# heli-sudoo/HKD-MPC

Hardware: NVIDIA B200
Metric: batched HS-DDP solves/sec (higher is better)
Workload: dtype f64

## Files before the change

### hkd-mpc_b200/__init__.py

```python
import ctypes as C
import os
import subprocess
import numpy as np

_HERE = os.path.dirname(os.path.abspath(__file__))
LIB_PATH = os.environ.get("HSDDP_LIB") or os.path.join(_HERE, "libhsddp_b200.so")

MAX_PHASES = 16
MAX_STAGES = 128
TRACE_CAP = 64

STATUS_NAMES = {0: "converged", 1: "stalled", 2: "max_iter", 3: "reg_overflow"}

ARR = dict(Xbar=0, X=1, Defect=3, dX=4, G0=5, Ubar=10, U=11, dU=12, K=20, A=21, B=22, lxx=24, luu=25, H0=27,
           lx=30, lu=31, h=50, al=51, g=52, reb=53)


class HsddpError(RuntimeError):

    def __init__(self, msg, code=None):
        super().__init__(msg)
        self.code = code


# ... 97 lines not shown
        L.hsddp_batch_mpc_update.argtypes = [vp]
        L.hsddp_batch_last_update_ms.argtypes = [vp, C.POINTER(C.c_float)]
        L.hsddp_batch_restart_problems.argtypes = [vp, C.c_int, ip, ip, ip, dp, C.POINTER(Options)]
        L.hsddp_batch_get_schedule_ids.argtypes = [vp, ip]
        for f in ("hsddp_batch_solve", "hsddp_batch_solve_async", "hsddp_batch_compute_cost", "hsddp_batch_lq_approximation",
                  "hsddp_batch_prepare_merit", "hsddp_batch_update_al_params", "hsddp_batch_update_reb_params"):
            getattr(L, f).argtypes = [vp, C.POINTER(Options)]
        L.hsddp_batch_sync.argtypes = [vp]
        L.hsddp_batch_update_nominal.argtypes = [vp]
        L.hsddp_batch_last_solve_ms.argtypes = [vp, C.POINTER(C.c_float)]
        L.hsddp_batch_hybrid_rollout.argtypes = [vp, C.c_double, C.POINTER(Options), ip]
        L.hsddp_batch_backward_sweep.argtypes = [vp, C.c_double, ip]
        L.hsddp_batch_backward_sweep_regularized.argtypes = [vp, dp, C.POINTER(Options), ip]
        L.hsddp_batch_linear_rollout.argtypes = [vp, C.c_double, C.POINTER(Options)]
        L.hsddp_batch_forward_sweep.argtypes = [vp, C.POINTER(Options), ip, dp]
        L.hsddp_batch_dims.argtypes = [vp, ip, ip, ip]
        L.hsddp_batch_get_info.argtypes = [vp, vp]
        L.hsddp_batch_get_trace.argtypes = [vp, dp]
        L.hsddp_batch_get_scalars.argtypes = [vp, dp]
        L.hsddp_batch_get_array.argtypes = [vp, C.c_int, dp]
        L.hsddp_batch_set_array.argtypes = [vp, C.c_int, dp]
        L.hsddp_fp64_peak_tflops.argtypes = [C.c_int, C.c_int, dp]
        L.hsddp_batch_get_array_rows.argtypes = [vp, C.c_int, C.c_int, C.c_int, dp]
        L.hsddp_batch_get_gains_compact.argtypes = [vp, C.c_int, C.c_int, dp]
        L.hsddp_batch_get_mpc_command.argtypes = [vp, C.c_int, vp]
        L.hsddp_batch_set_problems_from_gaits.argtypes = [vp, C.c_int, ip, C.POINTER(C.c_float), dp, dp, dp, dp, ip, C.c_int, ip, ip, C.c_float, C.c_int, ip,
                                                          C.POINTER(ConstraintParams)]
        L.hsddp_batch_get_schedule.argtypes = [vp, C.c_int, ip, ip, ip, ip, dp, dp, dp, dp]
        L.hsddp_batch_set_solve_mode.argtypes = [vp, C.c_int]
        L.hsddp_batch_event_record.argtypes = [vp, C.c_int]
        L.hsddp_batch_event_elapsed_ms.argtypes = [vp, C.c_int, C.c_int, C.POINTER(C.c_float)]
        L.hsddp_batch_get_counters.argtypes = [vp, C.POINTER(C.c_ulonglong)]
        L.hsddp_batch_reset_counters.argtypes = [vp]
        L.hsddp_batch_get_profile.argtypes = [vp, C.POINTER(C.c_ulonglong)]
        L.hsddp_phase_batch_create.argtypes = [C.c_int] * 6 + [C.POINTER(vp)]
        L.hsddp_phase_batch_destroy.argtypes = [vp]
        L.hsddp_phase_batch_set.argtypes = [vp, C.c_int, dp]
        L.hsddp_phase_batch_backward_sweep.argtypes = [vp, C.c_double, dp, dp, ip]
        L.hsddp_phase_batch_linear_rollout.argtypes = [vp, C.c_double, dp]
        L.hsddp_phase_batch_set_gains.argtypes = [vp, dp, dp]
        L.hsddp_phase_batch_get.argtypes = [vp, C.c_int, dp]
        L.hsddp_phase_batch_last_ms.argtypes = [vp, C.POINTER(C.c_float)]
        _lib = L
    return _lib


def _dp(a):
    return a.ctypes.data_as(C.POINTER(C.c_double))


def _ip(a):
    return a.ctypes.data_as(C.POINTER(C.c_int32))


def _fp(a):
    return a.ctypes.data_as(C.POINTER(C.c_float))


def _check(rc, what):
    if rc != 0:
        raise HsddpError(f"{what} failed with code {rc}: {lib().hsddp_last_error().decode()}", rc)


def model_dynamics(x, u, dt, contact):
    x = np.ascontiguousarray(x, np.float64); u = np.ascontiguousarray(u, np.float64)
    c = np.ascontiguousarray(contact, np.int32); xn = np.zeros(24)
# ... 251 lines not shown

    def get_rows(self, name, row0, nrows, out=None):
        cols = {"K": 576, "g": 20, "h": 4, "al": 16, "reb": 40}.get(name, 24)
        if out is None:
            out = np.zeros((self.n, nrows, cols))
        _check(lib().hsddp_batch_get_array_rows(self.h, ARR[name], int(row0), int(nrows), _dp(out)), "get_array_rows")
        return out

    def get_gains_compact(self, row0, nrows, out=None):
        if out is None:
            out = np.zeros((self.n, nrows, 24, 12))
        _check(lib().hsddp_batch_get_gains_compact(self.h, int(row0), int(nrows), _dp(out)), "get_gains_compact")
        return out

    def mpc_command(self, n_steps=8, out=None):
        if out is None:
            out = np.zeros(self.n, dtype=CMD_DTYPE)
        _check(lib().hsddp_batch_get_mpc_command(self.h, int(n_steps), out.ctypes.data_as(C.c_void_p)), "get_mpc_command")
        return out

    def event_record(self, slot):
        _check(lib().hsddp_batch_event_record(self.h, int(slot)), "event_record")

    def event_elapsed_ms(self, slot0, slot1):
        ms = C.c_float()
        _check(lib().hsddp_batch_event_elapsed_ms(self.h, int(slot0), int(slot1), C.byref(ms)), "event_elapsed_ms")
        return ms.value

    def counters(self):
        out = (C.c_ulonglong * 4)()
        _check(lib().hsddp_batch_get_counters(self.h, out), "get_counters")
        return dict(sweep_stages=int(out[0]), solve_launches=int(out[1]), step_launches=int(out[2]))

    def profile(self):
        out = (C.c_ulonglong * 16)()
        _check(lib().hsddp_batch_get_profile(self.h, out), "get_profile")
        return [int(v) for v in out]

    def reset_counters(self):
        _check(lib().hsddp_batch_reset_counters(self.h), "reset_counters")

    def set(self, name, arr):
        arr = np.ascontiguousarray(arr, np.float64)
        if name == "K":
            arr = np.ascontiguousarray(np.swapaxes(arr, -1, -2))
        _check(lib().hsddp_batch_set_array(self.h, ARR[name], _dp(arr)), "set_array")



class SinglePhaseBatch:
    INPUTS = ["A", "B", "C", "D", "lx", "lu", "ly", "lxx", "luu", "lux", "lyy", "Phix", "Phixx", "Defect"]
    OUTPUTS = ["dU", "K", "G", "H", "dX", "dV"]
    _MATS = {"A", "B", "C", "D", "lxx", "luu", "lux", "lyy", "Phixx", "K", "H"}

    def __init__(self, xs, us, ys, horizon, n_problems, device=0):
        self.xs, self.us, self.ys, self.N, self.n = int(xs), int(us), int(ys), int(horizon), int(n_problems)
        self.h = C.c_void_p()
        _check(lib().hsddp_phase_batch_create(int(device), self.xs, self.us, self.ys, self.N, self.n, C.byref(self.h)), "hsddp_phase_batch_create")

    def __del__(self):
        try:
            if self.h:
                lib().hsddp_phase_batch_destroy(self.h)
        except Exception:
            pass

# ... 53 lines not shown
```

### hkd-mpc_b200/csrc/hsddp_device.cuh

```cuda
#pragma once
#include <cuda_runtime.h>
#include <stdint.h>
#include <cstddef>
#include "../../include/hsddp_b200.h"
#include "hkd_model.cuh"

#ifdef HSDDP_PROFILE
#define PROF_DECL long long prof_t0_ = clock64();
#define PROF_MARK(sm, slot)                                                         \
    do {                                                                            \
        if (threadIdx.x == 0) {                                                     \
            const long long t1_ = clock64();                                        \
            (sm).profacc[slot] += (unsigned long long)(t1_ - prof_t0_);             \
            prof_t0_ = t1_;                                                         \
        }                                                                           \
    } while (0)
#else
#define PROF_DECL
#define PROF_MARK(sm, slot) do { } while (0)
#endif

namespace hsddp {

constexpr int kThreads = 128;
// ... 21 lines not shown
constexpr int TQ_JC = 124;
constexpr int TQ_STRIDE = 200;

struct DevSchedule {
    int n_phases, n_stages, n_nodes, _pad;
    int horizon[MAXPH];
    int node_off[MAXPH];
    int stage_off[MAXPH];
    unsigned cmask[MAXPH];
    unsigned nmask[MAXPH];
    long long ref_off;
    double dt;
    unsigned char ph_of_stage[HSDDP_MAX_STAGES];
    unsigned char ph_of_node[HSDDP_MAX_STAGES + MAXPH];
    unsigned char ss_size[MAXPH];
    unsigned char tdmask[2][MAXPH];
};
static_assert(sizeof(DevSchedule) % 4 == 0, "bind_problem copies the schedule word by word");

struct SolverState {
    double actual_cost, merit, feas, dV_1, dV_2;
    double max_tconstr_prev, max_pconstr_prev, max_tconstr, max_pconstr, merit_rho;
    double reg;
    int rollout_ok, sweep_ok;
};

struct SolveCtl {
    int iter, iter_ou, iter_in, n_sweeps, n_trials, status;
    int active;
    int have_trial;
    int max_al, max_ddp;
    double cost0, feas0;
    double trial_cost, trial_feas;
};

struct BatchPtrs {
    int n_problems, max_stages, max_nodes, _pad;
    const DevSchedule* sched;
    const int* sched_id;
    const double *xr, *ur, *prel, *xinit;
    double* x0;
    double *Xbar, *X, *Xsim_t, *Defect, *dX;
    double *Ubar, *U, *U_t, *dU;
    double* KdX;
    double* K;
    double* lq;
    double* tq;
    double* gcon;
    double* reb;
    double* hcon;
    double* al;
    double* g0h0;
    SolverState* state;
    SolveCtl* ctl;
    const int* active;
    const int* n_active;
    int* next_active;
    int* next_count;
    int* zero_count;
    int sweep_w1_min;
    int lr_external;
    int _pad2;
    double *ls_X, *ls_Defect, *ls_Xsim, *ls_U, *ls_Ut, *ls_gcon, *ls_hcon, *ls_res;
    int* ls_mail;
    const int* order;
    const int* budget;
    hsddp_info* info;
    hsddp_iter_record* trace;
    unsigned long long* counters;
    int* work_counter;
    int* sm_slots;
    hsddp_constraint_params cp;
};

struct Smem;
struct __align__(16) Smem {
    double H[ro(24)], Y[ro(24)];
    double Z[zo(24)];
    double Qux[ro(16) + kQuuPad];
    double Quu[ro(12)];
    double rec[2][LQ_STRIDE];
    double dfc2[2][24];
    double G[24], Gn[24], Qx[24], Qu[24], wu[24], vtmp[24], vtmp2[24];
    double lxxd[24], lxxTd[24], lxxw[12], lxxTw[12];
    double swdt[4];
    double swc[16];
    double red[kThreads];
    DevSchedule sc;
    SolverState st;
    SolveCtl ctl;
    hsddp_constraint_params cp;
    hsddp_options opt;
    double *Xbar, *X, *Xsim_t, *Defect, *dX, *Ubar, *U, *U_t, *dU, *KdX, *K, *lqg, *tq, *gcon, *reb, *hcon, *al, *g0h0;
    const double *xr, *ur, *prel, *xinit, *x0;
    unsigned long long* prof;
    unsigned long long profacc[16];
    int pid;
    int rot;
    int flag;
    int ibuf[4];
    double dbuf[8];
};

static_assert(offsetof(Smem, dfc2) - offsetof(Smem, H) == sizeof(double) * kSweepDoubles, "kSweepDoubles must cover H..rec");
static_assert(32 * 113 <= kSweepDoubles, "LQ staging buffer does not fit");
// ... 682 lines not shown
```

### hkd-mpc_b200/csrc/hsddp_kernels.cu

```cuda
#include <cuda_runtime.h>
#include <cooperative_groups.h>
#include <cstdio>
#include <cstdlib>
#include <cstring>
#include <string>
#include <vector>
#include <map>
#include <algorithm>
#include "hsddp_device.cuh"
#include "hsddp_sweep.cuh"
#include "hsddp_sweep_w1.cuh"
#include "hsddp_lr_w1.cuh"

#ifndef HSDDP_MIN_BLOCKS
#define HSDDP_MIN_BLOCKS 6
#endif

namespace hsddp {

constexpr int hsddp_batch_max_groups = 16;

__device__ inline void prepare_merit_block(Smem& sm) {
    if (threadIdx.x == 0) {
        SolverState& st = sm.st;
// ... 191 lines not shown
    if (tid == 0) { sm.ctl.cost0 = sm.st.actual_cost; sm.ctl.feas0 = sm.st.feas; }
    __syncthreads();
    if (sm.ctl.max_al <= 0) {
        if (tid == 0) sm.ctl.active = 0;
        __syncthreads();
        return;
    }
    outer_start_block(sm);
    if (sm.ctl.max_ddp <= 0) outer_end_block(sm);
}

__device__ inline void iter_prep_block(Smem& sm, const BatchPtrs& bp) {
    if (sm.ctl.have_trial) {
        if (threadIdx.x == 0) { sm.st.actual_cost = sm.ctl.trial_cost; sm.st.feas = sm.ctl.trial_feas; }
        __syncthreads();
    } else {
        compute_cost_block(sm);
    }
    if (threadIdx.x == 0) {
        sm.ctl.iter_in++; sm.ctl.iter++;
        if (sm.ctl.iter <= HSDDP_TRACE_CAP) {
            hsddp_iter_record rec;
            rec.outer = sm.ctl.iter_ou; rec.inner = sm.ctl.iter_in; rec.cost_before = sm.st.actual_cost; rec.feas_before = sm.st.feas;
            rec.reg_after = rec.n_sweeps = 0;
            rec.dV_1 = rec.dV_2 = rec.merit_rho = rec.eps_accepted = rec.n_trials = 0; rec._pad = 0;
            rec.cost_after = rec.feas_after = rec.max_tconstr = rec.max_pconstr = 0;
            bp.trace[(size_t)sm.pid * HSDDP_TRACE_CAP + sm.ctl.iter - 1] = rec;
        }
    }
    __syncthreads();
    lq_approximation_block(sm);
}

__device__ inline void iter_sweep_block(Smem& sm, const BatchPtrs& bp) {
    int nsw = 0;
    const bool success = backward_sweep_regularized_block(sm, nsw);
    if (threadIdx.x == 0) {
        sm.ctl.n_sweeps += nsw;
        if (sm.ctl.iter <= HSDDP_TRACE_CAP) {
            hsddp_iter_record& rec = bp.trace[(size_t)sm.pid * HSDDP_TRACE_CAP + sm.ctl.iter - 1];
            rec.n_sweeps = nsw; rec.reg_after = sm.st.reg;
        }
        if (!success) { sm.ctl.status = HSDDP_STATUS_REG_OVERFLOW; sm.ctl.active = 0; }
    }
    __syncthreads();
}

template <bool CLUSTER_LS = false>
__device__ inline void iter_forward_block(Smem& sm, const BatchPtrs& bp) {
    const int tid = threadIdx.x;
    const hsddp_options& opt = sm.opt;
    hsddp_iter_record* rec = (sm.ctl.iter <= HSDDP_TRACE_CAP) ? bp.trace + (size_t)sm.pid * HSDDP_TRACE_CAP + sm.ctl.iter - 1 : nullptr;
    if (opt.MS && !bp.lr_external) linear_rollout_block(sm, 1.0);
    prepare_merit_block(sm);
    const double cost_prev = sm.st.actual_cost, merit_prev = sm.st.merit;
    const double dV_abs = fabs(sm.st.dV_1 + 0.5 * sm.st.dV_2);
    bool leave_inner = false;
    if (tid == 0 && rec) { rec->dV_1 = sm.st.dV_1; rec->dV_2 = sm.st.dV_2; rec->merit_rho = sm.st.merit_rho; }
    if ((dV_abs < opt.cost_thresh) && (sm.st.feas <= opt.dynamics_feas_thresh)) {
        if (tid == 0 && rec) {
            rec->eps_accepted = -1; rec->n_trials = 0;
            rec->cost_after = sm.st.actual_cost; rec->feas_after = sm.st.feas; rec->max_tconstr = sm.st.max_tconstr; rec->max_pconstr = sm.st.max_pconstr;
        }
        leave_inner = true;
    } else {
        double eps_acc = 0;
        int ntr = 0;
        if (CLUSTER_LS ? line_search_cluster(sm, bp, eps_acc, ntr) : line_search_block<true>(sm, eps_acc, ntr)) {
            update_nominal_block(sm);
        } else {
            __syncthreads();
            if (tid == 0) { sm.st.actual_cost = cost_prev; sm.st.merit = merit_prev; }
            __syncthreads();
        }
        if (tid == 0) {
            sm.ctl.n_trials += ntr;
            if (rec) {
                rec->eps_accepted = eps_acc; rec->n_trials = ntr;
// ... 105 lines not shown
                const int c = *rl.count[g];
                if (q < c) { pid = rl.list[g][q]; break; }
                q -= c;
            }
            sm.ibuf[3] = pid;
        }
        __syncthreads();
        const int pid = sm.ibuf[3];
        if (pid < 0) break;
        bind_problem(sm, bp, pid);
        if (threadIdx.x == 0) sm.opt = opt;
        __syncthreads();
        while (sm.ctl.active) {
            iter_prep_block(sm, bp);
            iter_sweep_block(sm, bp);
            if (!sm.ctl.active) break;
            iter_forward_block(sm, bp);
        }
        solve_finish_block(sm, bp);
        if (threadIdx.x == 0) { bp.state[pid] = sm.st; bp.ctl[pid] = sm.ctl; }
    }
}

enum SolvePhase { PH_BEGIN = 0, PH_PREP, PH_SWEEP, PH_FORWARD };
#ifndef HSDDP_MINB_SWEEP
#define HSDDP_MINB_SWEEP 5
#endif
#ifndef HSDDP_MINB_OTHER
#define HSDDP_MINB_OTHER 6
#endif
template <int PH>
__global__ void __launch_bounds__(kThreads, PH == 2 ? HSDDP_MINB_SWEEP : HSDDP_MINB_OTHER) k_phase(BatchPtrs bp, hsddp_options opt) {
    __shared__ Smem sm;
    if (PH == PH_PREP && bp.zero_count && blockIdx.x == 0 && threadIdx.x == 0) *bp.zero_count = 0;
    if (bp.n_active && (int)blockIdx.x >= *bp.n_active) return;
    if (PH == PH_SWEEP && bp.n_active && bp.sweep_w1_min > 0 && *bp.n_active >= bp.sweep_w1_min) return;
    const int pid = bp.active ? bp.active[blockIdx.x] : (int)blockIdx.x;
    if (threadIdx.x == 0) assign_rotation(bp.sm_slots, sm.rot);
    bind_problem(sm, bp, pid);
    if (threadIdx.x == 0) sm.opt = opt;
    __syncthreads();
#ifdef HSDDP_PROFILE
    if (threadIdx.x == 0) for (int i = 0; i < 16; ++i) sm.profacc[i] = 0;
    __syncthreads();
#endif
    if (PH == PH_BEGIN) solve_begin_block(sm, bp);
    if (PH == PH_PREP) iter_prep_block(sm, bp);
    if (PH == PH_SWEEP) iter_sweep_block(sm, bp);
    if (PH == PH_FORWARD) {
        if (sm.ctl.active) iter_forward_block(sm, bp);
    }
    __syncthreads();
    if (PH == PH_BEGIN || PH == PH_FORWARD) {
        if (sm.ctl.active) {
            if (threadIdx.x == 0) bp.next_active[atomicAdd(bp.next_count, 1)] = pid;
        } else {
            solve_finish_block(sm, bp);
        }
    }
    if (threadIdx.x == 0) { bp.state[pid] = sm.st; bp.ctl[pid] = sm.ctl; }
#ifdef HSDDP_PROFILE
    if (threadIdx.x == 0) for (int i = 0; i < 16; ++i) atomicAdd(&sm.prof[i], sm.profacc[i]);
#endif
}

enum StepOp { OP_RESET = 0, OP_ROLLOUT, OP_COST, OP_LQ, OP_SWEEP, OP_SWEEP_REG, OP_LINEAR, OP_MERIT, OP_FORWARD, OP_NOMINAL, OP_AL, OP_REB };

__global__ void __launch_bounds__(kThreads, HSDDP_MIN_BLOCKS) k_step(BatchPtrs bp, hsddp_options opt, int op, double arg, double* darg, int* ok) {
    __shared__ Smem sm;
    const int pid = blockIdx.x;
    if (threadIdx.x == 0) assign_rotation(bp.sm_slots, sm.rot);
    bind_problem(sm, bp, pid);
    if (threadIdx.x == 0) sm.opt = opt;
    __syncthreads();
    int okv = 1;
    switch (op) {
        case OP_RESET: cold_start_block(sm); break;
        case OP_ROLLOUT: okv = hybrid_rollout_block<false>(sm, arg) ? 1 : 0; break;
        case OP_COST: compute_cost_block(sm); break;
        case OP_LQ: lq_approximation_block(sm); break;
        case OP_SWEEP: okv = backward_sweep_block(sm, arg) ? 1 : 0; break;
        case OP_SWEEP_REG: {
            if (threadIdx.x == 0) sm.st.reg = darg[pid];
            __syncthreads();
            int nsw;
            okv = backward_sweep_regularized_block(sm, nsw) ? 1 : 0;
            if (threadIdx.x == 0) darg[pid] = sm.st.reg;
        } break;
        case OP_LINEAR: linear_rollout_block(sm, arg); break;
        case OP_MERIT: prepare_merit_block(sm); break;
        case OP_FORWARD: {
            const double cost_prev = sm.st.actual_cost, merit_prev = sm.st.merit;
            double eps_acc; int ntr;
// ... 440 lines not shown
namespace hsddp { void set_last_error(const std::string& s) { g_last_error = s; } }

#define CK(call)                                                                                   \
    do {                                                                                           \
        cudaError_t e_ = (call);                                                                   \
        if (e_ != cudaSuccess) {                                                                   \
            g_last_error = std::string(#call) + ": " + cudaGetErrorString(e_);                     \
            return HSDDP_ERR_CUDA;                                                                 \
        }                                                                                          \
    } while (0)

struct hsddp_batch {
    int device = 0;
    cudaStream_t stream = nullptr;
    cudaEvent_t ev0 = nullptr, ev1 = nullptr;
    cudaEvent_t slots[8] = {nullptr, nullptr, nullptr, nullptr, nullptr, nullptr, nullptr, nullptr};
    unsigned long long n_solve_launches = 0, n_step_launches = 0;
    int n_sm = 0, blocks_per_sm = 1;
    BatchPtrs bp{};
    std::vector<void*> allocs;
    std::vector<DevSchedule> h_sched;
    std::vector<int> h_sched_id;
    bool has_problems = false;
    bool cold = true;
    float last_ms = 0.f;
    int* d_ok = nullptr;
    double* d_darg = nullptr;
    int solve_mode = 0;
    int* d_active[2] = {nullptr, nullptr};
    int* d_count = nullptr;
    int last_rounds = 0;
    int sweep_kind = 2;
    int w1_min_blocks = 1036;
    bool lr_w1 = true;
    int* d_order = nullptr;
    bool have_order = false, use_order = true;
    bool cluster_ls = true;
    static constexpr int kClusterLsMax = 32;
    static constexpr int kMaxGroups = 16;
    int phased_min_group = 1024;
    int hybrid_rounds = 20, hybrid_groups = 4, hybrid_min_group = 256;
    int phased_groups = 4;
    cudaStream_t gstream[kMaxGroups] = {};
    cudaEvent_t gevent[kMaxGroups] = {};
    cudaEvent_t ev_fork = nullptr;
    hsddp_mpc_command* d_cmd = nullptr;
    bool mpc_ready = false;
    GaitLib lib{};
    int *d_sched_gait = nullptr, *d_sched_window = nullptr, *d_mpc_err = nullptr;
    MpcSched* d_mpc = nullptr;
    float plan = 0.f;
    int node_stride = 0, n_sched = 0;
    bool h_sched_stale = false;
    cudaEvent_t ev_u0 = nullptr, ev_u1 = nullptr;
    int n_gaits = 0;
    std::vector<int> slot_refs;
    std::vector<int> slot_free;
    int* d_restart = nullptr;
    double* d_restart_x0 = nullptr;
    size_t d_restart_cap = 0, d_restart_x0_cap = 0;
    int* d_budget = nullptr;
    long long budget_rounds = -1;
    bool slots_marked = false;
};

namespace {
// ... 108 lines not shown
        {(void**)&b->d_darg, 1, D, -1, 0},
    };
}

bool stored_array(hsddp_batch* b, int which, WsArray* out) {
    if (which < 0) return false;
    for (const WsArray& a : workspace_arrays(b))
        if (a.abi == which) { *out = a; return true; }
    return false;
}

struct SlotArray { void** field; size_t bytes; };

std::vector<SlotArray> slot_arrays(hsddp_batch* b) {
    BatchPtrs& bp = b->bp;
    const size_t rows = (size_t)b->node_stride, D = sizeof(double);
    return {
        {(void**)&bp.sched, sizeof(DevSchedule)}, {(void**)&b->d_mpc, sizeof(MpcSched)},
        {(void**)&b->d_sched_gait, sizeof(int)}, {(void**)&b->d_sched_window, sizeof(int)},
        {(void**)&bp.xr, 24 * rows * D}, {(void**)&bp.ur, 24 * rows * D}, {(void**)&bp.prel, 12 * rows * D}, {(void**)&bp.xinit, 24 * rows * D},
    };
}

void free_problem_allocs(hsddp_batch* b) {
    for (void* p : b->allocs) cudaFree(p);
    b->allocs.clear();
    b->d_cmd = nullptr;
    b->has_problems = false;
    b->mpc_ready = false;
    b->h_sched_stale = false;
    b->slot_refs.clear(); b->slot_free.clear();
    b->d_restart = nullptr; b->d_restart_x0 = nullptr; b->d_restart_cap = b->d_restart_x0_cap = 0;
    b->d_budget = nullptr; b->budget_rounds = -1;
    b->slots_marked = false;
}

hsddp_options default_options() {
    hsddp_options o;
    std::memset(&o, 0, sizeof o);
    o.alpha = 0.1; o.gamma = 0.01; o.update_penalty = 5; o.update_relax = 1; o.update_regularization = 2; o.update_ReB = 1;
    o.max_DDP_iter = 10; o.max_AL_iter = 5; o.cost_thresh = 1e-3; o.tconstr_thresh = 1e-3; o.pconstr_thresh = 1e-3;
    o.dynamics_feas_thresh = 1e-3; o.merit_scale = 0.2; o.merit_offset = 1e2; o.AL_active = 1; o.ReB_active = 1; o.MS = 1;
    return o;
}

const char* check_budget(int max_AL_iter, int max_DDP_iter) {
    if (max_DDP_iter < 0 || max_AL_iter < 0) return "max_DDP_iter / max_AL_iter must be >= 0";
    if ((long long)max_DDP_iter * (long long)max_AL_iter > 1000000LL) return "max_DDP_iter x max_AL_iter exceeds 1e6";
    return nullptr;
}

int check_opt(const hsddp_options* opt) {
    if (!opt) return HSDDP_OK;
    auto fin = [](double v) { return v == v && v - v == 0.0; };
    const char* bad = nullptr;
    if (!(opt->alpha > 0.0 && opt->alpha < 1.0)) bad = "alpha must be in (0, 1)";
    else if (!(opt->update_regularization > 1.0) || !fin(opt->update_regularization)) bad = "update_regularization must be finite and > 1";
    else if (!fin(opt->gamma) || !fin(opt->update_penalty) || !fin(opt->update_relax) || !fin(opt->update_ReB)) bad = "gamma / update_penalty / update_relax / update_ReB must be finite";
    else if (!fin(opt->cost_thresh) || !fin(opt->tconstr_thresh) || !fin(opt->pconstr_thresh) || !fin(opt->dynamics_feas_thresh)) bad = "thresholds must be finite";
    else if (!fin(opt->merit_scale) || opt->merit_scale == 1.0 || !fin(opt->merit_offset)) bad = "merit_scale must be finite and != 1, merit_offset finite";
    else bad = check_budget(opt->max_AL_iter, opt->max_DDP_iter);
    if (bad) { g_last_error = std::string("invalid hsddp_options: ") + bad; return HSDDP_ERR_ARG; }
    return HSDDP_OK;
}

int launch_step(hsddp_batch* b, const hsddp_options* opt, int op, double arg, double* darg_dev, int32_t* ok_host, bool sync = true) {
// ... 15 lines not shown

extern "C" {

static int batch_init(hsddp_batch* b, int device) {
    CK(cudaSetDevice(device));
    b->device = device;
    CK(cudaStreamCreateWithFlags(&b->stream, cudaStreamNonBlocking));
    CK(cudaEventCreate(&b->ev0));
    CK(cudaEventCreate(&b->ev1));
    CK(cudaEventCreate(&b->ev_u0));
    CK(cudaEventCreate(&b->ev_u1));
    for (int i = 0; i < 8; ++i) CK(cudaEventCreate(&b->slots[i]));
    cudaDeviceProp prop;
    CK(cudaGetDeviceProperties(&prop, device));
    b->n_sm = prop.multiProcessorCount;
    CK(cudaOccupancyMaxActiveBlocksPerMultiprocessor(&b->blocks_per_sm, k_solve, kThreads, 0));
    if (b->blocks_per_sm < 1) b->blocks_per_sm = 1;
    if (const char* e = getenv("HSDDP_BLOCKS_PER_SM")) {
        const int v = atoi(e);
        if (v >= 1 && v <= b->blocks_per_sm) b->blocks_per_sm = v;
    }
    CK(cudaEventCreateWithFlags(&b->ev_fork, cudaEventDisableTiming));
    if (const char* e = getenv("HSDDP_PHASED_GROUPS")) {
        const int v = atoi(e);
        if (v >= 1 && v <= hsddp_batch::kMaxGroups) b->phased_groups = v;
    }
    if (const char* e = getenv("HSDDP_PHASED_MIN_GROUP")) { const int v = atoi(e); if (v >= 1) b->phased_min_group = v; }
    if (const char* e = getenv("HSDDP_HYBRID_ROUNDS")) b->hybrid_rounds = atoi(e);
    if (const char* e = getenv("HSDDP_HYBRID_GROUPS")) { const int v = atoi(e); if (v >= 1 && v <= hsddp_batch::kMaxGroups) b->hybrid_groups = v; }
    if (const char* e = getenv("HSDDP_SWEEP_KIND")) b->sweep_kind = atoi(e);
    CK(cudaFuncSetAttribute(k_sweep_w1, cudaFuncAttributePreferredSharedMemoryCarveout, cudaSharedmemCarveoutMaxShared));
    CK(cudaFuncSetAttribute(k_lr_w1, cudaFuncAttributePreferredSharedMemoryCarveout, cudaSharedmemCarveoutMaxShared));
    if (const char* e = getenv("HSDDP_W1_MIN_BLOCKS")) b->w1_min_blocks = atoi(e);
    if (const char* e = getenv("HSDDP_LR_W1")) b->lr_w1 = atoi(e) != 0;
    if (const char* e = getenv("HSDDP_QUEUE_ORDER")) b->use_order = atoi(e) != 0;
    if (const char* e = getenv("HSDDP_CLUSTER_LS")) b->cluster_ls = atoi(e) != 0;
    if (const char* e = getenv("HSDDP_SOLVE_MODE")) {
        const int v = atoi(e);
        if (v >= 0 && v <= 3) b->solve_mode = v;
    }
    return HSDDP_OK;
}

int hsddp_batch_create(int device, hsddp_batch** out) {
    if (!out) return HSDDP_ERR_ARG;
    *out = nullptr;
    int n = 0;
    CK(cudaGetDeviceCount(&n));
    if (device < 0 || device >= n) { g_last_error = "no such CUDA device (this library has no CPU fallback)"; return HSDDP_ERR_CUDA; }
    return guarded([&]() -> int {
        hsddp_batch* b = new hsddp_batch();
        const int rc = batch_init(b, device);
        if (rc != HSDDP_OK) { hsddp_batch_destroy(b); return rc; }
        *out = b;
        return HSDDP_OK;
    });
}

int hsddp_batch_destroy(hsddp_batch* b) {
    if (!b) return HSDDP_OK;
    cudaSetDevice(b->device);
    free_problem_allocs(b);
    if (b->ev0) cudaEventDestroy(b->ev0);
    if (b->ev1) cudaEventDestroy(b->ev1);
    if (b->ev_u0) cudaEventDestroy(b->ev_u0);
    if (b->ev_u1) cudaEventDestroy(b->ev_u1);
// ... 398 lines not shown
    const int work = 33 * q.n_iter + 48 * q.n_sweeps + 12 * q.n_trials;
    return 255 - min(max(work >> 6, 0), 255);
}
__global__ void k_order_by_iterations(const hsddp_info* info, int n, int* order) {
    __shared__ int bins[256], start[256];
    for (int i = threadIdx.x; i < 256; i += blockDim.x) bins[i] = 0;
    __syncthreads();
    for (int i = threadIdx.x; i < n; i += blockDim.x) atomicAdd(&bins[order_bin(info[i])], 1);
    __syncthreads();
    if (threadIdx.x == 0) {
        int acc = 0;
        for (int i = 0; i < 256; ++i) { start[i] = acc; acc += bins[i]; }
    }
    __syncthreads();
    for (int bi = threadIdx.x; bi < 256; bi += blockDim.x) {
        if (!bins[bi]) continue;
        int pos = start[bi];
        for (int i = 0; i < n; ++i)
            if (order_bin(info[i]) == bi) order[pos++] = i;
    }
}

static int solve_phased(hsddp_batch* b, const hsddp_options& o, bool hybrid) {
    const int P = b->bp.n_problems;
    int G = hybrid ? b->hybrid_groups : b->phased_groups;
    G = std::min(G, std::max(1, P / (hybrid ? b->hybrid_min_group : b->phased_min_group)));
    G = std::max(1, std::min(G, hsddp_batch::kMaxGroups));
    for (int g = 0; g < G; ++g) {
        if (!b->gstream[g]) {
            CK(cudaStreamCreateWithFlags(&b->gstream[g], cudaStreamNonBlocking));
            CK(cudaEventCreateWithFlags(&b->gevent[g], cudaEventDisableTiming));
        }
    }
    CK(cudaEventRecord(b->ev0, b->stream));
    CK(cudaMemsetAsync(b->d_count, 0, 2 * hsddp_batch::kMaxGroups * sizeof(int), b->stream));
    k_iota<<<(P + 255) / 256, 256, 0, b->stream>>>(b->d_active[0], P);
    CK(cudaEventRecord(b->ev_fork, b->stream));
    const int all_rounds = (int)std::min<long long>(std::max((long long)std::max(0, o.max_AL_iter) * (long long)std::max(0, o.max_DDP_iter), b->budget_rounds), 1000000LL);
    const int rounds = hybrid ? std::min(all_rounds, std::max(0, b->hybrid_rounds)) : all_rounds;
    ResumeLists rl{};
    rl.n = 0;
    const bool use_block = b->sweep_kind != 1, use_w1 = b->sweep_kind != 0;
    int rc = HSDDP_OK;
    for (int g = 0; g < G && rc == HSDDP_OK; ++g) {
        const int lo = (int)((long long)P * g / G), n = (int)((long long)P * (g + 1) / G) - lo;
        if (n <= 0) continue;
        cudaStream_t st = b->gstream[g];
        int* cnt[2] = {b->d_count + 2 * g, b->d_count + 2 * g + 1};
        int* list[2] = {b->d_active[0] + lo, b->d_active[1] + lo};
        if (cudaStreamWaitEvent(st, b->ev_fork, 0) != cudaSuccess) { rc = HSDDP_ERR_CUDA; break; }
        BatchPtrs bp = b->bp;
        bp.sweep_w1_min = b->sweep_kind == 0 ? 0 : b->sweep_kind == 1 ? 1 : b->w1_min_blocks;
        bp.lr_external = (b->lr_w1 && o.MS) ? 1 : 0;
        bp.active = list[0]; bp.n_active = nullptr; bp.next_active = list[1]; bp.next_count = cnt[1]; bp.zero_count = nullptr;
        k_phase<PH_BEGIN><<<n, kThreads, 0, st>>>(bp, o);
        b->n_solve_launches++;
        for (int r = 1; r <= rounds; ++r) {
            const int cur = r & 1;
            bp.active = list[cur]; bp.n_active = cnt[cur]; bp.next_active = list[cur ^ 1]; bp.next_count = cnt[cur ^ 1]; bp.zero_count = cnt[cur ^ 1];
            k_phase<PH_PREP><<<n, kThreads, 0, st>>>(bp, o);
            if (use_block) k_phase<PH_SWEEP><<<n, kThreads, 0, st>>>(bp, o);
            if (use_w1) k_sweep_w1<<<n, 32, 0, st>>>(bp, o);
            if (bp.lr_external) k_lr_w1<<<n, 32, 0, st>>>(bp, o);
            k_phase<PH_FORWARD><<<n, kThreads, 0, st>>>(bp, o);
            b->n_solve_launches += 3 + (use_block && use_w1 ? 1 : 0) + (bp.lr_external ? 1 : 0);
        }
        if (cudaGetLastError() != cudaSuccess) { rc = HSDDP_ERR_CUDA; g_last_error = "kernel launch failed in the phased driver"; }
        const int nxt = (rounds + 1) & 1;
        rl.list[rl.n] = list[nxt]; rl.count[rl.n] = cnt[nxt]; rl.n++;
    }
    b->last_rounds = rounds;
    for (int g = 0; g < G; ++g) {
        if (!b->gstream[g]) continue;
        if (cudaEventRecord(b->gevent[g], b->gstream[g]) == cudaSuccess) cudaStreamWaitEvent(b->stream, b->gevent[g], 0);
    }
    if (hybrid && rounds < all_rounds && rc == HSDDP_OK) {
        CK(cudaMemsetAsync(b->bp.work_counter, 0, sizeof(int), b->stream));
        k_solve_resume<4><<<b->n_sm * 4, kThreads, 0, b->stream>>>(b->bp, o, rl);
        CK(cudaGetLastError());
        b->n_solve_launches++;
    }
    CK(cudaEventRecord(b->ev1, b->stream));
    return rc;
}

int hsddp_batch_set_solve_mode(hsddp_batch* b, int mode) {
    if (!b || mode < 0 || mode > 3) return HSDDP_ERR_ARG;
    b->solve_mode = mode;
    return HSDDP_OK;
}

static int consume_budget(hsddp_batch* b) {
    if (b->budget_rounds < 0) return HSDDP_OK;
    CK(cudaMemsetAsync(b->d_budget, 0xff, sizeof(int) * 2 * b->bp.n_problems, b->stream));
// ... 268 lines not shown
    }
    k_command<<<b->bp.n_problems, 128, 0, b->stream>>>(b->bp, n_steps, b->d_cmd);
    CK(cudaGetLastError());
    b->n_step_launches++;
    CK(cudaMemcpyAsync(out, b->d_cmd, bytes, cudaMemcpyDeviceToHost, b->stream));
    CK(cudaStreamSynchronize(b->stream));
    return HSDDP_OK;
}

int hsddp_batch_event_record(hsddp_batch* b, int slot) {
    if (!b || slot < 0 || slot >= 8) return HSDDP_ERR_ARG;
    CK(cudaSetDevice(b->device));
    CK(cudaEventRecord(b->slots[slot], b->stream));
    return HSDDP_OK;
}

int hsddp_batch_event_elapsed_ms(hsddp_batch* b, int slot0, int slot1, float* ms) {
    if (!b || !ms || slot0 < 0 || slot0 >= 8 || slot1 < 0 || slot1 >= 8) return HSDDP_ERR_ARG;
    CK(cudaSetDevice(b->device));
    CK(cudaEventSynchronize(b->slots[slot1]));
    CK(cudaEventElapsedTime(ms, b->slots[slot0], b->slots[slot1]));
    return HSDDP_OK;
}

int hsddp_batch_get_counters(hsddp_batch* b, unsigned long long out[4]) {
    if (!b || !b->has_problems || !out) return HSDDP_ERR_ARG;
    CK(cudaSetDevice(b->device));
    CK(cudaStreamSynchronize(b->stream));
    CK(cudaMemcpy(out, b->bp.counters, sizeof(unsigned long long), cudaMemcpyDeviceToHost));
    out[1] = b->n_solve_launches; out[2] = b->n_step_launches; out[3] = 0;
    return HSDDP_OK;
}

int hsddp_batch_get_profile(hsddp_batch* b, unsigned long long out[16]) {
    if (!b || !b->has_problems || !out) return HSDDP_ERR_ARG;
    CK(cudaSetDevice(b->device));
    CK(cudaStreamSynchronize(b->stream));
    CK(cudaMemcpy(out, b->bp.counters + 8, 16 * sizeof(unsigned long long), cudaMemcpyDeviceToHost));
    return HSDDP_OK;
}

int hsddp_batch_reset_counters(hsddp_batch* b) {
    if (!b || !b->has_problems) return HSDDP_ERR_ARG;
    CK(cudaSetDevice(b->device));
    CK(cudaMemsetAsync(b->bp.counters, 0, 32 * sizeof(unsigned long long), b->stream));
    b->n_solve_launches = 0; b->n_step_launches = 0;
    return HSDDP_OK;
}

int hsddp_fp64_peak_tflops(int device, int kind, double* tflops) {
    if (!tflops) return HSDDP_ERR_ARG;
    CK(cudaSetDevice(device));
    cudaDeviceProp prop;
    CK(cudaGetDeviceProperties(&prop, device));
    const int blocks = prop.multiProcessorCount * 8, threads = 256, iters = 20000;
    double* d = nullptr;
    CK(cudaMalloc(&d, sizeof(double) * blocks * threads));
    cudaEvent_t e0, e1;
    CK(cudaEventCreate(&e0));
    CK(cudaEventCreate(&e1));
    double best = 0;
    for (int rep = 0; rep < 4; ++rep) {
        CK(cudaEventRecord(e0));
        if (kind == 0) k_dfma_probe<<<blocks, threads>>>(d, iters);
        else k_dmma_probe<<<blocks, threads>>>(d, iters);
        CK(cudaEventRecord(e1));
// ... 16 lines not shown
```

### include/hsddp_b200.h

```cpp
#ifndef HSDDP_B200_H
#define HSDDP_B200_H

#include <stdint.h>

#ifdef __cplusplus
extern "C" {
#endif

#define HSDDP_NX 24
#define HSDDP_NU 24
#define HSDDP_MAX_PHASES 16
#define HSDDP_MAX_STAGES 128

#define HSDDP_OK 0
#define HSDDP_ERR_ARG (-1)
#define HSDDP_ERR_CUDA (-2)
#define HSDDP_ERR_UNSUPPORTED (-3)
#define HSDDP_ERR_STATE (-4)
#define HSDDP_ERR_IO (-5)

#define HSDDP_STATUS_CONVERGED 0
#define HSDDP_STATUS_STALLED 1
#define HSDDP_STATUS_MAX_ITER 2
#define HSDDP_STATUS_REG_OVERFLOW 3
// ... 119 lines not shown
#define HSDDP_ARR_LU 31
#define HSDDP_ARR_LUU 25
#define HSDDP_ARR_LXX 24
#define HSDDP_ARR_G0 5
#define HSDDP_ARR_H0 27
#define HSDDP_ARR_GCON 52
#define HSDDP_ARR_HCON 50
#define HSDDP_ARR_AL 51
#define HSDDP_ARR_REB 53
int hsddp_batch_get_array(hsddp_batch* b, int which, double* out);
int hsddp_batch_set_array(hsddp_batch* b, int which, const double* in);

int hsddp_batch_get_array_rows(hsddp_batch* b, int which, int row0, int nrows, double* out);

int hsddp_batch_get_gains_compact(hsddp_batch* b, int row0, int nrows, double* out);

#define HSDDP_CMD_MAX_STEPS 10
typedef struct hsddp_mpc_command {
    int32_t N_mpcsteps;
    int32_t foot_found[4];
    int32_t contacts[HSDDP_CMD_MAX_STEPS][4];
    float hkd_controls[HSDDP_CMD_MAX_STEPS][24];
    float des_body_state[HSDDP_CMD_MAX_STEPS][12];
    float feedback[HSDDP_CMD_MAX_STEPS][12][12];
    float foot_placement[12];
    int32_t _pad;
} hsddp_mpc_command;
int hsddp_batch_get_mpc_command(hsddp_batch* b, int n_steps, hsddp_mpc_command* out);

int hsddp_batch_event_record(hsddp_batch* b, int slot);
int hsddp_batch_event_elapsed_ms(hsddp_batch* b, int slot0, int slot1, float* ms);
int hsddp_batch_get_counters(hsddp_batch* b, unsigned long long out[4]);
int hsddp_batch_reset_counters(hsddp_batch* b);
int hsddp_batch_get_profile(hsddp_batch* b, unsigned long long out[16]);

typedef struct hsddp_phase_batch hsddp_phase_batch;
#define HSDDP_PH_A 0
#define HSDDP_PH_B 1
#define HSDDP_PH_C 2
#define HSDDP_PH_D 3
#define HSDDP_PH_LX 4
#define HSDDP_PH_LU 5
#define HSDDP_PH_LY 6
#define HSDDP_PH_LXX 7
#define HSDDP_PH_LUU 8
#define HSDDP_PH_LUX 9
#define HSDDP_PH_LYY 10
#define HSDDP_PH_PHIX 11
#define HSDDP_PH_PHIXX 12
#define HSDDP_PH_DEFECT 13
#define HSDDP_PH_N_INPUTS 14
#define HSDDP_PH_OUT_DU 0
#define HSDDP_PH_OUT_K 1
#define HSDDP_PH_OUT_G 2
#define HSDDP_PH_OUT_H 3
#define HSDDP_PH_OUT_DX 4
#define HSDDP_PH_OUT_DV 5
#define HSDDP_PH_N_OUTPUTS 6
int hsddp_phase_batch_create(int device, int xs, int us, int ys, int horizon, int n_problems, hsddp_phase_batch** out);
int hsddp_phase_batch_destroy(hsddp_phase_batch* b);
int hsddp_phase_batch_set(hsddp_phase_batch* b, int which, const double* host);
int hsddp_phase_batch_backward_sweep(hsddp_phase_batch* b, double regularization, const double* Gprime, const double* Hprime, int32_t* ok);
int hsddp_phase_batch_linear_rollout(hsddp_phase_batch* b, double eps, const double* dx_init);
int hsddp_phase_batch_set_gains(hsddp_phase_batch* b, const double* dU, const double* K);
int hsddp_phase_batch_get(hsddp_phase_batch* b, int which, double* host);
int hsddp_phase_batch_last_ms(hsddp_phase_batch* b, float* ms);
// ... 8 lines not shown
```

Measured before the change: 57150.

## Speculatively run regularization retries of backward sweep in parallel blocks

Problems likely to need regularization retries (nonzero reg or multiple sweeps last iteration) are flagged in the prep phase. The sweep kernel then launches extra blocks, each running the backward sweep at a higher candidate regularization level into scratch buffers. The last block to arrive picks the first successful candidate and copies its gains back. This turns serial retry sweeps into parallel ones, at the cost of extra blocks per round, scratch memory and atomics, and redundant work when the base sweep succeeds.

Measured after the change: 58950, median of 6. 1.03x the previous value.

```diff
diff --git a/hkd-mpc_b200/__init__.py b/hkd-mpc_b200/__init__.py
--- a/hkd-mpc_b200/__init__.py
+++ b/hkd-mpc_b200/__init__.py
@@ -153,6 +153,7 @@
         L.hsddp_batch_event_elapsed_ms.argtypes = [vp, C.c_int, C.c_int, C.POINTER(C.c_float)]
         L.hsddp_batch_get_counters.argtypes = [vp, C.POINTER(C.c_ulonglong)]
         L.hsddp_batch_reset_counters.argtypes = [vp]
+        L.hsddp_batch_get_speculation.argtypes = [vp, C.POINTER(C.c_ulonglong)]
         L.hsddp_batch_get_profile.argtypes = [vp, C.POINTER(C.c_ulonglong)]
         L.hsddp_phase_batch_create.argtypes = [C.c_int] * 6 + [C.POINTER(vp)]
         L.hsddp_phase_batch_destroy.argtypes = [vp]
@@ -470,6 +471,11 @@
         _check(lib().hsddp_batch_get_counters(self.h, out), "get_counters")
         return dict(sweep_stages=int(out[0]), solve_launches=int(out[1]), step_launches=int(out[2]))
 
+    def speculation(self):
+        out = (C.c_ulonglong * 3)()
+        _check(lib().hsddp_batch_get_speculation(self.h, out), "get_speculation")
+        return dict(rounds=int(out[0]), later=int(out[1]), exceeded=int(out[2]))
+
     def profile(self):
         out = (C.c_ulonglong * 16)()
         _check(lib().hsddp_batch_get_profile(self.h, out), "get_profile")
diff --git a/hkd-mpc_b200/csrc/hsddp_device.cuh b/hkd-mpc_b200/csrc/hsddp_device.cuh
--- a/hkd-mpc_b200/csrc/hsddp_device.cuh
+++ b/hkd-mpc_b200/csrc/hsddp_device.cuh
@@ -77,6 +77,11 @@
     int max_al, max_ddp;
     double cost0, feas0;
     double trial_cost, trial_feas;
+};
+
+struct SpecRec {
+    int ok, _pad;
+    double dV_1, dV_2;
 };
 
 struct BatchPtrs {
@@ -116,6 +121,14 @@
     int* work_counter;
     int* sm_slots;
     hsddp_constraint_params cp;
+    int* spec_list;
+    int* spec_count;
+    int* spec_zero;
+    int* spec_arrive;
+    int* spec_entry;
+    SpecRec* spec_rec;
+    double* spec_out;
+    int spec_S, spec_cap;
 };
 
 struct Smem;
diff --git a/hkd-mpc_b200/csrc/hsddp_kernels.cu b/hkd-mpc_b200/csrc/hsddp_kernels.cu
--- a/hkd-mpc_b200/csrc/hsddp_kernels.cu
+++ b/hkd-mpc_b200/csrc/hsddp_kernels.cu
@@ -247,9 +247,7 @@
     lq_approximation_block(sm);
 }
 
-__device__ inline void iter_sweep_block(Smem& sm, const BatchPtrs& bp) {
-    int nsw = 0;
-    const bool success = backward_sweep_regularized_block(sm, nsw);
+__device__ inline void finish_sweep_block(Smem& sm, const BatchPtrs& bp, bool success, int nsw) {
     if (threadIdx.x == 0) {
         sm.ctl.n_sweeps += nsw;
         if (sm.ctl.iter <= HSDDP_TRACE_CAP) {
@@ -259,6 +257,119 @@
         if (!success) { sm.ctl.status = HSDDP_STATUS_REG_OVERFLOW; sm.ctl.active = 0; }
     }
     __syncthreads();
+}
+
+__device__ inline void iter_sweep_block(Smem& sm, const BatchPtrs& bp) {
+    int nsw = 0;
+    const bool success = backward_sweep_regularized_block(sm, nsw);
+    finish_sweep_block(sm, bp, success, nsw);
+}
+
+__device__ __forceinline__ bool retry_reg(double& r, int j, double up) {
+    for (int i = 0; i < j; ++i) {
+        r = fmax(r * up, 1e-03);
+        if (r > 1e2) return false;
+    }
+    return true;
+}
+
+__device__ inline void spec_flag_block(Smem& sm, const BatchPtrs& bp) {
+    if (threadIdx.x == 0) {
+        const int row = sm.ctl.iter - 1;
+        bool flag = sm.st.reg > 0;
+        if (row >= 1 && row <= HSDDP_TRACE_CAP) flag = flag || bp.trace[(size_t)sm.pid * HSDDP_TRACE_CAP + row - 1].n_sweeps > 1;
+        int e = -1;
+        if (flag) {
+            e = atomicAdd(bp.spec_count, 1);
+            if (e < bp.spec_cap) bp.spec_list[e] = sm.pid;
+            else e = -1;
+        }
+        bp.spec_entry[sm.pid] = e;
+    }
+}
+
+constexpr unsigned long long kSpecUnwritten = 0x7ff0dead5eed0001ull;
+
+__device__ inline bool spec_commit_block(Smem& sm, const BatchPtrs& bp, int e, int j, bool ran, bool ok, double& reg, int& nsw, bool& success) {
+    const int tid = threadIdx.x, S = bp.spec_S, N = sm.sc.n_stages;
+    const size_t ms = (size_t)bp.max_stages, slice = ms * 312 + 600;
+    SpecRec* rec = bp.spec_rec + (size_t)e * S;
+    const double* out = bp.spec_out + (size_t)e * (S - 1) * slice;
+    if (tid == 0) rec[j] = SpecRec{ran ? (ok ? 1 : 0) : -1, 0, sm.st.dV_1, sm.st.dV_2};
+    __threadfence();
+    __syncthreads();
+    if (tid == 0) sm.ibuf[2] = atomicAdd(bp.spec_arrive + e, 1) == S - 1;
+    __syncthreads();
+    if (!sm.ibuf[2]) return false;
+    __threadfence();
+    if (tid == 0) {
+        bp.spec_arrive[e] = 0;
+        int w = -1, m = 0;
+        while (m < S) {
+            const int c = __ldcg(&rec[m].ok);
+            if (c < 0) break;
+            ++m;
+            if (c) { w = m - 1; break; }
+        }
+        const int c = w >= 0 ? w : m - 1;
+        sm.ibuf[2] = w; sm.ibuf[3] = m;
+        const size_t pid = (size_t)sm.pid;
+        sm.K = bp.K + pid * ms * 288; sm.dU = bp.dU + pid * ms * 24; sm.g0h0 = bp.g0h0 + pid * 600;
+        sm.st.dV_1 = __ldcg(&rec[c].dV_1); sm.st.dV_2 = __ldcg(&rec[c].dV_2); sm.st.sweep_ok = w >= 0 ? 1 : 0;
+        atomicAdd(bp.counters + 1, 1ull);
+        if (w != 0) atomicAdd(bp.counters + (w > 0 ? 2 : 3), 1ull);
+    }
+    __syncthreads();
+    const int w = sm.ibuf[2], m = sm.ibuf[3];
+    for (int c = (w >= 0 ? w : 1); c <= (w >= 0 ? w : m - 1); ++c) {
+        if (c == 0) continue;
+        const double* o = out + (c - 1) * slice;
+        const unsigned long long* mark = reinterpret_cast<const unsigned long long*>(o + ms * 288);
+        for (int x = tid; x < 288 * N; x += kThreads)
+            if (w >= 0 || __ldcg(mark + 24 * (x / 288)) != kSpecUnwritten) sm.K[x] = __ldcg(o + x);
+        for (int x = tid; x < 24 * N; x += kThreads)
+            if (w >= 0 || __ldcg(mark + 24 * (x / 24)) != kSpecUnwritten) sm.dU[x] = __ldcg(o + ms * 288 + x);
+        if (w >= 0)
+            for (int x = tid; x < 600; x += kThreads) sm.g0h0[x] = __ldcg(o + ms * 312 + x);
+        __syncthreads();
+    }
+    success = w >= 0;
+    nsw = success ? w + 1 : m;
+    reg = sm.st.reg;
+    retry_reg(reg, success ? w : m - 1, sm.opt.update_regularization);
+    return true;
+}
+
+__device__ inline bool sweep_round_block(Smem& sm, const BatchPtrs& bp, int e, int j) {
+    const int tid = threadIdx.x;
+    const double up = sm.opt.update_regularization;
+    double reg = sm.st.reg;
+    int nsw = 0;
+    bool success = false, run = e < 0 || retry_reg(reg, j, up);
+    if (e >= 0 && j > 0 && run) {
+        const size_t ms = (size_t)bp.max_stages;
+        double* o = bp.spec_out + ((size_t)e * (bp.spec_S - 1) + j - 1) * (ms * 312 + 600);
+        for (int s = tid; s < sm.sc.n_stages; s += kThreads) reinterpret_cast<unsigned long long*>(o + ms * 288)[24 * s] = kSpecUnwritten;
+        if (tid == 0) { sm.K = o; sm.dU = o + ms * 288; sm.g0h0 = o + ms * 312; }
+    }
+    __syncthreads();
+    for (;;) {
+        if (run) { ++nsw; success = backward_sweep_block(sm, reg); }
+        if (e >= 0) {
+            if (!spec_commit_block(sm, bp, e, j, run, success, reg, nsw, success)) return false;
+            e = -1;
+        }
+        if (success) break;
+        reg = fmax(reg * up, 1e-03);
+        if (reg > 1e2) break;
+        run = true;
+    }
+    reg = reg / 20;
+    if (reg < 1e-06) reg = 0;
+    if (tid == 0) sm.st.reg = reg;
+    __syncthreads();
+    finish_sweep_block(sm, bp, success, nsw);
+    return true;
 }
 
 template <bool CLUSTER_LS = false>
@@ -430,10 +541,20 @@
 template <int PH>
 __global__ void __launch_bounds__(kThreads, PH == 2 ? HSDDP_MINB_SWEEP : HSDDP_MINB_OTHER) k_phase(BatchPtrs bp, hsddp_options opt) {
     __shared__ Smem sm;
-    if (PH == PH_PREP && bp.zero_count && blockIdx.x == 0 && threadIdx.x == 0) *bp.zero_count = 0;
-    if (bp.n_active && (int)blockIdx.x >= *bp.n_active) return;
+    if (PH == PH_PREP && bp.zero_count && blockIdx.x == 0 && threadIdx.x == 0) {
+        *bp.zero_count = 0;
+        if (bp.spec_zero) *bp.spec_zero = 0;
+    }
+    int blk = (int)blockIdx.x, cand = 0, entry = -1;
+    if (PH == PH_SWEEP && bp.spec_list) {
+        const int ns = bp.spec_cap * (bp.spec_S - 1);
+        if (blk < ns) { entry = blk / (bp.spec_S - 1); cand = 1 + blk % (bp.spec_S - 1); }
+        blk -= ns;
+    }
+    if (bp.n_active && blk >= *bp.n_active) return;
     if (PH == PH_SWEEP && bp.n_active && bp.sweep_w1_min > 0 && *bp.n_active >= bp.sweep_w1_min) return;
-    const int pid = bp.active ? bp.active[blockIdx.x] : (int)blockIdx.x;
+    if (PH == PH_SWEEP && cand > 0 && entry >= min(*bp.spec_count, bp.spec_cap)) return;
+    const int pid = cand > 0 ? bp.spec_list[entry] : bp.active ? bp.active[blk] : blk;
     if (threadIdx.x == 0) assign_rotation(bp.sm_slots, sm.rot);
     bind_problem(sm, bp, pid);
     if (threadIdx.x == 0) sm.opt = opt;
@@ -442,9 +563,16 @@
     if (threadIdx.x == 0) for (int i = 0; i < 16; ++i) sm.profacc[i] = 0;
     __syncthreads();
 #endif
+    bool store = true;
     if (PH == PH_BEGIN) solve_begin_block(sm, bp);
-    if (PH == PH_PREP) iter_prep_block(sm, bp);
-    if (PH == PH_SWEEP) iter_sweep_block(sm, bp);
+    if (PH == PH_PREP) {
+        iter_prep_block(sm, bp);
+        if (bp.spec_list && (bp.sweep_w1_min == 0 || *bp.n_active < bp.sweep_w1_min)) spec_flag_block(sm, bp);
+    }
+    if (PH == PH_SWEEP) {
+        if (bp.spec_list && cand == 0) entry = bp.spec_entry[pid];
+        store = sweep_round_block(sm, bp, entry, cand);
+    }
     if (PH == PH_FORWARD) {
         if (sm.ctl.active) iter_forward_block(sm, bp);
     }
@@ -456,7 +584,7 @@
             solve_finish_block(sm, bp);
         }
     }
-    if (threadIdx.x == 0) { bp.state[pid] = sm.st; bp.ctl[pid] = sm.ctl; }
+    if (store && threadIdx.x == 0) { bp.state[pid] = sm.st; bp.ctl[pid] = sm.ctl; }
 #ifdef HSDDP_PROFILE
     if (threadIdx.x == 0) for (int i = 0; i < 16; ++i) atomicAdd(&sm.prof[i], sm.profacc[i]);
 #endif
@@ -963,6 +1091,12 @@
     int last_rounds = 0;
     int sweep_kind = 2;
     int w1_min_blocks = 1036;
+    int sweep_spec = 8;
+    static constexpr int kSpecCap = 128;
+    int* d_spec_int = nullptr;
+    SpecRec* d_spec_rec = nullptr;
+    double* d_spec_out = nullptr;
+    size_t d_spec_int_cap = 0, d_spec_rec_cap = 0, d_spec_out_cap = 0;
     bool lr_w1 = true;
     int* d_order = nullptr;
     bool have_order = false, use_order = true;
@@ -1137,6 +1271,7 @@
     b->slot_refs.clear(); b->slot_free.clear();
     b->d_restart = nullptr; b->d_restart_x0 = nullptr; b->d_restart_cap = b->d_restart_x0_cap = 0;
     b->d_budget = nullptr; b->budget_rounds = -1;
+    b->d_spec_int = nullptr; b->d_spec_rec = nullptr; b->d_spec_out = nullptr; b->d_spec_int_cap = b->d_spec_rec_cap = b->d_spec_out_cap = 0;
     b->slots_marked = false;
 }
 
@@ -1218,6 +1353,7 @@
     CK(cudaFuncSetAttribute(k_sweep_w1, cudaFuncAttributePreferredSharedMemoryCarveout, cudaSharedmemCarveoutMaxShared));
     CK(cudaFuncSetAttribute(k_lr_w1, cudaFuncAttributePreferredSharedMemoryCarveout, cudaSharedmemCarveoutMaxShared));
     if (const char* e = getenv("HSDDP_W1_MIN_BLOCKS")) b->w1_min_blocks = atoi(e);
+    if (const char* e = getenv("HSDDP_SWEEP_SPEC")) { const int v = atoi(e); b->sweep_spec = (v >= 2 && v <= 32) ? v : 0; }
     if (const char* e = getenv("HSDDP_LR_W1")) b->lr_w1 = atoi(e) != 0;
     if (const char* e = getenv("HSDDP_QUEUE_ORDER")) b->use_order = atoi(e) != 0;
     if (const char* e = getenv("HSDDP_CLUSTER_LS")) b->cluster_ls = atoi(e) != 0;
@@ -1682,15 +1818,24 @@
             CK(cudaEventCreateWithFlags(&b->gevent[g], cudaEventDisableTiming));
         }
     }
+    const bool use_block = b->sweep_kind != 1, use_w1 = b->sweep_kind != 0;
+    const int S = use_block && b->sweep_spec > 1 ? b->sweep_spec : 0, cap = hsddp_batch::kSpecCap;
+    const size_t slice = (size_t)b->bp.max_stages * 312 + 600, spec_ints = (size_t)G * (2 * cap + 2) + P;
+    if (S) {
+        int rs = scratch(b, &b->d_spec_int, &b->d_spec_int_cap, spec_ints);
+        if (!rs) rs = scratch(b, &b->d_spec_rec, &b->d_spec_rec_cap, (size_t)G * cap * S);
+        if (!rs) rs = scratch(b, &b->d_spec_out, &b->d_spec_out_cap, (size_t)G * cap * (S - 1) * slice);
+        if (rs) return rs;
+    }
     CK(cudaEventRecord(b->ev0, b->stream));
     CK(cudaMemsetAsync(b->d_count, 0, 2 * hsddp_batch::kMaxGroups * sizeof(int), b->stream));
+    if (S) CK(cudaMemsetAsync(b->d_spec_int, 0, spec_ints * sizeof(int), b->stream));
     k_iota<<<(P + 255) / 256, 256, 0, b->stream>>>(b->d_active[0], P);
     CK(cudaEventRecord(b->ev_fork, b->stream));
     const int all_rounds = (int)std::min<long long>(std::max((long long)std::max(0, o.max_AL_iter) * (long long)std::max(0, o.max_DDP_iter), b->budget_rounds), 1000000LL);
     const int rounds = hybrid ? std::min(all_rounds, std::max(0, b->hybrid_rounds)) : all_rounds;
     ResumeLists rl{};
     rl.n = 0;
-    const bool use_block = b->sweep_kind != 1, use_w1 = b->sweep_kind != 0;
     int rc = HSDDP_OK;
     for (int g = 0; g < G && rc == HSDDP_OK; ++g) {
         const int lo = (int)((long long)P * g / G), n = (int)((long long)P * (g + 1) / G) - lo;
@@ -1705,11 +1850,18 @@
         bp.active = list[0]; bp.n_active = nullptr; bp.next_active = list[1]; bp.next_count = cnt[1]; bp.zero_count = nullptr;
         k_phase<PH_BEGIN><<<n, kThreads, 0, st>>>(bp, o);
         b->n_solve_launches++;
+        int* spec = b->d_spec_int + (size_t)g * (2 * cap + 2);
+        if (S) {
+            bp.spec_list = spec; bp.spec_arrive = spec + cap; bp.spec_entry = b->d_spec_int + (size_t)G * (2 * cap + 2);
+            bp.spec_rec = b->d_spec_rec + (size_t)g * cap * S; bp.spec_out = b->d_spec_out + (size_t)g * cap * (S - 1) * slice;
+            bp.spec_S = S; bp.spec_cap = cap;
+        }
         for (int r = 1; r <= rounds; ++r) {
             const int cur = r & 1;
             bp.active = list[cur]; bp.n_active = cnt[cur]; bp.next_active = list[cur ^ 1]; bp.next_count = cnt[cur ^ 1]; bp.zero_count = cnt[cur ^ 1];
+            if (S) { bp.spec_count = spec + 2 * cap + cur; bp.spec_zero = spec + 2 * cap + (cur ^ 1); }
             k_phase<PH_PREP><<<n, kThreads, 0, st>>>(bp, o);
-            if (use_block) k_phase<PH_SWEEP><<<n, kThreads, 0, st>>>(bp, o);
+            if (use_block) k_phase<PH_SWEEP><<<n + (S ? cap * (S - 1) : 0), kThreads, 0, st>>>(bp, o);
             if (use_w1) k_sweep_w1<<<n, 32, 0, st>>>(bp, o);
             if (bp.lr_external) k_lr_w1<<<n, 32, 0, st>>>(bp, o);
             k_phase<PH_FORWARD><<<n, kThreads, 0, st>>>(bp, o);
@@ -2044,6 +2196,14 @@
     return HSDDP_OK;
 }
 
+int hsddp_batch_get_speculation(hsddp_batch* b, unsigned long long out[3]) {
+    if (!b || !b->has_problems || !out) return HSDDP_ERR_ARG;
+    CK(cudaSetDevice(b->device));
+    CK(cudaStreamSynchronize(b->stream));
+    CK(cudaMemcpy(out, b->bp.counters + 1, 3 * sizeof(unsigned long long), cudaMemcpyDeviceToHost));
+    return HSDDP_OK;
+}
+
 int hsddp_batch_get_profile(hsddp_batch* b, unsigned long long out[16]) {
     if (!b || !b->has_problems || !out) return HSDDP_ERR_ARG;
     CK(cudaSetDevice(b->device));
diff --git a/include/hsddp_b200.h b/include/hsddp_b200.h
--- a/include/hsddp_b200.h
+++ b/include/hsddp_b200.h
@@ -175,6 +175,7 @@
 int hsddp_batch_event_elapsed_ms(hsddp_batch* b, int slot0, int slot1, float* ms);
 int hsddp_batch_get_counters(hsddp_batch* b, unsigned long long out[4]);
 int hsddp_batch_reset_counters(hsddp_batch* b);
+int hsddp_batch_get_speculation(hsddp_batch* b, unsigned long long out[3]);
 int hsddp_batch_get_profile(hsddp_batch* b, unsigned long long out[16]);
 
 typedef struct hsddp_phase_batch hsddp_phase_batch;
```
